# MarSaKi/VLN-BEVBert

Hardware: AMD Instinct MI355X
Metric: pretrain_samples_per_sec (higher is better)
Workload: dtype bf16+fp32-residual

## Files before the change

### include/bevbert_hip.h

```cpp
#ifndef BEVBERT_HIP_H
#define BEVBERT_HIP_H

#include <stdint.h>

#ifdef __cplusplus
extern "C" {
#endif

typedef struct ihipStream_t* hipStream_t;

#define BEVBERT_F32 0
#define BEVBERT_BF16 1
#define BEVBERT_F16 2

const char* bevbert_last_error(void);
int bevbert_version(void);
int bevbert_hip_error_reset(void);
const char* bevbert_arch(void);
const char* bevbert_attn_last_path(int backward);
const char* bevbert_attn_plan(int B, int nh, int Lq, int Lk, int dtype, int impl, int has_key_mask, int has_bias,
                              float drop_p, int has_bits, int bits_ready, int want_dbias, int ncu, int backward);

int bevbert_bev_lift_bin(const float* depths, const float* T_c2w, const float* T_w2c, const float* S_w2c,
                         const float* pix_scale, int B, int V, int hw, float depth_scale, int dim, float res,
// ... 38 lines not shown
                                const float* gamma, const float* beta, void* y16, float* y32, float* z32, float* mean,
                                float* rstd, int rows, int H, float eps, float drop_p, uint64_t seed, uint64_t offset,
                                hipStream_t stream);
int bevbert_layernorm_res32_bwd(const void* dy16, const float* dy32, const float* z32, const float* mean,
                                const float* rstd, const float* gamma, void* dz, void* dx16, float* dgamma,
                                float* dbeta, float* dbias, float* workspace, int rows, int H, float drop_p, uint64_t seed,
                                uint64_t offset, int accumulate, int dz_dtype,
                                hipStream_t stream);
int64_t bevbert_colsum_workspace_floats(int total_cols);
int bevbert_colsum_partial_rows(int rows);
int bevbert_colsum_finalize(const float* partials, int nblocks, int nwhich, int C, float* out0, float* out1,
                            float* out2, int accumulate, hipStream_t stream);
int bevbert_colsum_partials(const void* dy, float* partials, int rows, int C, int dtype, hipStream_t stream);
int bevbert_multi_finalize(const void* tasks, int ntasks, hipStream_t stream);
int bevbert_multi_accum(const void* tasks, int ntasks, hipStream_t stream);

int bevbert_embed_sum_layernorm_fwd(const int64_t* ids, const void* word, const void* pos, const void* type_row,
                                    const float* gamma, const float* beta, void* y, void* z_out, float* mean,
                                    float* rstd, int rows, int L, int H, float eps, int dtype, float drop_p,
                                    uint64_t seed, uint64_t offset, hipStream_t stream);

int bevbert_embedding_grad(const int64_t* ids, const void* d, float* table_grad, int rows, int H, int padding_idx,
                           int dtype, hipStream_t stream);

int64_t bevbert_smallk_workspace_floats(int rows, int K, int H);
int bevbert_smallk_linear_layernorm_fwd(const float* feat, const float* weight, const float* bias, const float* gamma,
                                        const float* beta, const void* post1, const void* table, const int64_t* idx,
                                        void* y, float* mean, float* rstd, int rows, int K, int H, float eps, int dtype,
                                        hipStream_t stream);
int bevbert_smallk_linear_layernorm_bwd(const void* dy, const float* feat, const float* weight, const float* bias,
// ... 28 lines not shown

int bevbert_bias_gelu_fwd(const void* x, const float* bias, void* y, int rows, int C, int dtype, hipStream_t stream);
int bevbert_bias_gelu_bwd(const void* dy, const void* x, const float* bias, void* dx, float* dbias, float* workspace,
                          int rows, int C, int dtype, int accumulate, hipStream_t stream);
int bevbert_bias_relu_fwd(const void* x, const float* bias, void* y, int rows, int C, int dtype, hipStream_t stream);
int bevbert_bias_relu_bwd(const void* dy, const void* x, const float* bias, void* dx, float* dbias, float* workspace,
                          int rows, int C, int dtype, int accumulate, hipStream_t stream);
int bevbert_colsum(const void* dy, float* out, float* workspace, int rows, int C, int dtype, int accumulate,
                   hipStream_t stream);

int bevbert_segment_wsum(const void* src, const int* rowptr, const int* idx, const float* w, void* out, int out_rows,
                         int H, int dtype, hipStream_t stream);

int bevbert_grad_norm_clip(const float* grads, int64_t n, float pre_scale, float max_norm, float* partials,
                           float* scalars, hipStream_t stream);
int bevbert_adamw_step(float* params, const float* grads, float* exp_avg, float* exp_avg_sq, void* params_bf16,
                       const uint8_t* chunk_flags, int* chunk_steps, int64_t n, const float* grad_scale_dev,
                       const float* lr_dev, float lr, float beta1, float beta2, float eps, float weight_decay,
                       hipStream_t stream);
int bevbert_cast_f32(const float* src, void* dst, int64_t n, int dst_dtype, hipStream_t stream);
int bevbert_zero(void* p, int64_t bytes, hipStream_t stream);
int bevbert_accum_partials(const void* partials, float* sink, int S, int64_t n, int dtype, hipStream_t stream);

int bevbert_gemm(const void* A, const void* B, void* C, const void* bias, int M, int N, int K, int opA, int opB,
                 int64_t lda, int64_t ldb, int64_t ldc, int batch, int64_t stride_a, int64_t stride_b,
                 int64_t stride_c, int in_dtype, int out_dtype, int bias_dtype, float alpha, void* workspace,
                 int64_t workspace_bytes, int autotune, hipStream_t stream);
int bevbert_gemm_plan(int M, int N, int K, int opA, int opB, int64_t lda, int64_t ldb, int64_t ldc, int batch,
                      int64_t stride_a, int64_t stride_b, int64_t stride_c, int in_dtype, int out_dtype, int bias_dtype,
                      int accumulate, int64_t workspace_bytes, int autotune);
// ... 216 lines not shown
```

### vln_bevbert_amd/arena.py

```python
import math

import torch

from . import lib
from .lib import ptr, stream


def call(name, *args):
    from . import ops
    return ops.call(name, *args)

CHUNK = 1024
_ZERO_KERNEL = __import__("os").environ.get("BEVBERT_ZERO_KERNEL", "0") == "1"
NO_DECAY = ("bias", "LayerNorm.bias", "LayerNorm.weight")


def _round_up(n, m):
    return (n + m - 1) // m * m


class ParamArena:
    def __init__(self, module, device, compute_dtype=torch.float32, groups=()):
        self.device = torch.device(device)
        self.compute_dtype = compute_dtype
        named = [(n, p) for n, p in module.named_parameters()]
        by_name = dict(named)
        in_group = {}
        for gi, g in enumerate(groups):
            for n in g:
                in_group[n] = gi
        layout, seen_groups = [], set()
        for n, p in named:
            if n in in_group:
                gi = in_group[n]
                if gi in seen_groups:
                    continue
# ... 43 lines not shown
        self._param_versions = None
        self.step_count = 0
        self._scalars = torch.zeros(4, dtype=torch.float32, device=dev)
        self._partials = torch.zeros(1024, dtype=torch.float32, device=dev)
        self.named = named
        for n, p in named:
            o, k = self.slices[n]
            view = self.params[o:o + k].view(p.shape)
            view.copy_(p.data.to(dev, torch.float32))
            p.data = view
            p.main_grad = self.grads[o:o + k].view(p.shape)
            p.compute = self.shadow[o:o + k].view(p.shape) if self.shadow is not None else p.data
            p.arena = self
            p.arena_name = n
        self._index = {n: i for i, (n, _) in enumerate(named)}
        self.sync_shadow()
        self._param_versions = sum(p._version for _, p in named)

    def packed(self, names, shape):
        o0, _ = self.slices[names[0]]
        total = 0
        for n in names:
            o, k = self.slices[n]
            assert o == o0 + total, f"{names} are not contiguous in the arena"
            total += k
        assert total == math.prod(shape)
        src = self.shadow if self.shadow is not None else self.params
        return src[o0:o0 + total].view(shape), self.grads[o0:o0 + total].view(shape)

    def touch(self, param):
# ... 61 lines not shown
        if self.shadow is not None:
            call("bevbert_cast_f32", ptr(self.params), ptr(self.shadow), self.numel, lib.dtype_code(self.compute_dtype),
                 stream())

    def sync(self):
        if self.device.type == "cuda":
            from . import ops
            ops.WgradStream.flush_all()
            cur = torch.cuda.current_stream(self.device)
            for side in ops.Branches.side_streams():
                if ops.Branches.enabled or side not in ops.WgradStream.streams or ops.WgradStream.dirty:
                    cur.wait_stream(side)
            ops.WgradStream.dirty = False
            ops.WgradStream.release()

    def backward_done(self):
        self.sync()

    def zero_grad(self, overlap=False):
        self.sync()
        if self.device.type == "cuda":
            from . import ops
            ops.RT.scratch.reset()
            if overlap:
                if getattr(self, "_zero_stream", None) is None:
                    from .hwqueues import side_stream
                    self._zero_stream = side_stream(self.device)
                self._zero_stream.wait_stream(torch.cuda.current_stream(self.device))
                with torch.cuda.stream(self._zero_stream):
                    if _ZERO_KERNEL:
                        self.grads.zero_()
                    else:
                        call("bevbert_zero", ptr(self.grads), self.grads.numel() * 4, stream())
                self._zero_pending = True
                return
            call("bevbert_zero", ptr(self.grads), self.grads.numel() * 4, stream())
            return
        self.grads.zero_()
# ... 5 lines not shown

    def load_state_dict_into(self, module, sd, strict=True):
        out = module.load_state_dict(sd, strict=strict)
        self.sync_shadow()
        return out

    def set_lr(self, lr):
        self._scalars[2:3].fill_(float(lr))
        self._lr_set = True

    def upload_flags(self):
        if self._flags_dirty:
            self.flags.copy_(self._flags_host, non_blocking=True)
            self._flags_dirty = False

    def clip_and_step(self, lr=None, betas=(0.9, 0.98), eps=1e-6, weight_decay=0.01, max_norm=5.0, grad_pre_scale=1.0):
        self.sync()
        if self.exp_avg is None:
            self.exp_avg = torch.zeros_like(self.params)
            self.exp_avg_sq = torch.zeros_like(self.params)
        if lr is not None:
            self.set_lr(lr)
        elif not getattr(self, "_lr_set", False):
            raise RuntimeError("clip_and_step(lr=None) reads the device-resident learning rate: call set_lr() first "
                               "(the slot starts at 0, which would silently turn AdamW and its weight decay into a no-op)")
        if not torch.cuda.is_current_stream_capturing():
            self.upload_flags()
        self.step_count += 1
        call("bevbert_grad_norm_clip", ptr(self.grads), self.numel, float(grad_pre_scale),
             float(max_norm if max_norm is not None else -1.0), ptr(self._partials), ptr(self._scalars), stream())
        call("bevbert_adamw_step", ptr(self.params), ptr(self.grads), ptr(self.exp_avg), ptr(self.exp_avg_sq),
             ptr(self.shadow), ptr(self.flags), ptr(self.chunk_steps), self.numel, self._scalars[1:].data_ptr(),
             self._scalars[2:].data_ptr(), 0.0, float(betas[0]), float(betas[1]), float(eps), float(weight_decay),
             stream())

    def grad_norm(self):
        return self._scalars[0]
```

### vln_bevbert_amd/csrc/capi.hip

```cpp
#include <stdarg.h>

#include "attn_common.h"

static thread_local char g_err[512] = "";

void bb_set_error(const char* fmt, ...) {
  va_list ap;
  va_start(ap, fmt);
  vsnprintf(g_err, sizeof(g_err), fmt, ap);
  va_end(ap);
}

BEVBERT_API const char* bevbert_last_error(void) { return g_err; }
BEVBERT_API int bevbert_hip_error_reset(void) {
  int n = 0;
  while (hipGetLastError() != hipSuccess && n < 16) ++n;
  return n;
}

BEVBERT_API int bevbert_zero(void* p, int64_t bytes, hipStream_t stream) {
  BB_REQUIRE(p != nullptr && bytes >= 0, "zero: null pointer or negative size");
  if (bytes == 0) return BB_OK;
  hipError_t e = hipMemsetAsync(p, 0, (size_t)bytes, stream);
  if (e != hipSuccess) {
    bb_set_error("zero: hipMemsetAsync failed: %s", hipGetErrorString(e));
    return BB_ELAUNCH;
  }
  return BB_OK;
}

BEVBERT_API int bevbert_version(void) { return 205; }

static const uint32_t* g_step_salt = nullptr;
const uint32_t* bb_step_salt() { return g_step_salt; }
BEVBERT_API int bevbert_set_step_salt(const void* device_word) {
  g_step_salt = static_cast<const uint32_t*>(device_word);
  return BB_OK;
}
BEVBERT_API const char* bevbert_arch(void) { return "gfx950"; }

int attn_simple_fwd(const AttnArgs& a, int dtype, hipStream_t st);
int attn_simple_bwd(const AttnArgs& a, int dtype, hipStream_t st);
int attn_delta(const AttnArgs& a, float* delta, int dtype, hipStream_t st);
int attn_mfma_fwd(const AttnArgs& a, hipStream_t st);
int attn_mfma_bwd(const AttnArgs& a, hipStream_t st);
int attn_mfma_bwd1(const AttnArgs& a, hipStream_t st);
bool attn_mfma_bwd1_supported(const AttnArgs& a);
int attn_fwd2(const AttnArgs& a, hipStream_t st);
bool attn_fwd2_supported(const AttnArgs& a);
int attn_drop_bits(const AttnArgs& a, uint64_t* bits_f, uint64_t* bits_b, uint32_t* bits_l, hipStream_t st);
int attn_fwd4(const AttnArgs& a, const uint32_t* bits_l, hipStream_t st);
// ... 259 lines not shown
```

### vln_bevbert_amd/csrc/common.h

```cpp
#pragma once
#include <hip/hip_runtime.h>
#include <hip/hip_bf16.h>
#include <stdint.h>
#include <stdio.h>
#include <string.h>
#include <type_traits>

#include "../../include/bevbert_hip.h"

#define BEVBERT_API extern "C" __attribute__((visibility("default")))

enum { BB_F32 = BEVBERT_F32, BB_BF16 = BEVBERT_BF16, BB_F16 = BEVBERT_F16 };

enum { BB_OK = 0, BB_EINVAL = -1, BB_ELAUNCH = -2, BB_EUNSUPPORTED = -3 };

void bb_set_error(const char* fmt, ...);

#define BB_REQUIRE(cond, ...)            \
  do {                                   \
    if (!(cond)) {                       \
      bb_set_error(__VA_ARGS__);         \
      return BB_EINVAL;                  \
    }                                    \
  } while (0)
// ... 134 lines not shown
__host__ __device__ __forceinline__ uint32_t bb_site_key(uint64_t seed, uint64_t offset) {
  uint32_t k = bb_hash32((uint32_t)seed ^ 0x9e3779b9u);
  k = bb_hash32(k ^ (uint32_t)(seed >> 32));
  k = bb_hash32(k ^ (uint32_t)offset);
  return bb_hash32(k ^ (uint32_t)(offset >> 32));
}
constexpr uint32_t BB_STREAM_NAV = 0x6e617631u, BB_STREAM_WAYPOINT = 0x77617970u, BB_STREAM_GHOST = 0x67687374u;
constexpr uint32_t BB_STREAM_CE_ACTION = 0x63656163u;
__host__ __device__ __forceinline__ uint32_t bb_stream_key(uint32_t key, uint32_t domain) { return bb_hash32(key ^ domain); }
__host__ __device__ __forceinline__ uint32_t bb_drop_threshold(float p) {
  const float t = p * 65536.0f + 0.5f;
  if (t <= 0.f) return 0u;
  return t >= 65535.f ? 65535u : (uint32_t)t;
}
const uint32_t* bb_step_salt();
__device__ __forceinline__ uint32_t bb_salted(uint32_t key, const uint32_t* __restrict__ salt) {
  return salt ? bb_hash32(key ^ *salt) : key;
}
__device__ __forceinline__ uint32_t bb_pair_bits(uint32_t key, uint32_t pair_idx) { return bb_hash32(pair_idx ^ key); }
__device__ __forceinline__ bool bb_keep_lo(uint32_t bits, uint32_t thr) { return (bits & 0xffffu) >= thr; }
__device__ __forceinline__ bool bb_keep_hi(uint32_t bits, uint32_t thr) { return (bits >> 16) >= thr; }
__device__ __forceinline__ bool bb_keep(uint32_t key, uint32_t idx, uint32_t thr) {
  const uint32_t bits = bb_pair_bits(key, idx >> 1);
  return ((idx & 1u) ? (bits >> 16) : (bits & 0xffffu)) >= thr;
}
__device__ __forceinline__ float4 bb_drop4(float4 v, uint32_t elem, uint32_t key, uint32_t thr, float keep_scale) {
  const uint32_t pr = elem >> 1;
  const uint32_t b0 = bb_pair_bits(key, pr), b1 = bb_pair_bits(key, pr + 1);
  v.x = bb_keep_lo(b0, thr) ? v.x * keep_scale : 0.f;
  v.y = bb_keep_hi(b0, thr) ? v.y * keep_scale : 0.f;
// ... 66 lines not shown
```

### vln_bevbert_amd/csrc/rowops.hip

```cpp
#include <math.h>
#include <type_traits>

#include "common.h"

__device__ __forceinline__ float4 ln_fwd_input(float4 a, const float* __restrict__ bias, int col, float drop_p, uint32_t elem,
                                               uint32_t drop_key, uint32_t drop_thr, float keep_scale, bool has_res,
                                               const float4 r) {
  if (bias != nullptr) add4(a, *reinterpret_cast<const float4*>(bias + col));
  if (drop_p > 0.f) a = bb_drop4(a, elem, drop_key, drop_thr, keep_scale);
  if (has_res) add4(a, r);
  return a;
}

template <typename T, int NV, bool GATHER>
__global__ __launch_bounds__(256) void ln_fwd_kernel(const T* __restrict__ x, const float* __restrict__ bias,
                                                     const T* __restrict__ residual, const float* __restrict__ gamma,
                                                     const float* __restrict__ beta, T* __restrict__ y,
                                                     T* __restrict__ z_out, float* __restrict__ mean_out,
                                                     float* __restrict__ rstd_out, int rows, float eps, float drop_p,
                                                     uint32_t drop_thr, uint32_t drop_key,
                                                     const int64_t* __restrict__ ids, const T* __restrict__ word,
                                                     const T* __restrict__ pos, const T* __restrict__ type_row, int L,
                                                     const uint32_t* __restrict__ salt) {
  constexpr int H = NV * 256;
// ... 529 lines not shown
  const int r = blockIdx.x;
  const int e0 = rowptr[r], e1 = rowptr[r + 1];
  for (int c = threadIdx.x * 4; c < H; c += blockDim.x * 4) {
    float4 acc = make_float4(0.f, 0.f, 0.f, 0.f);
    for (int e = e0; e < e1; ++e) {
      const float ww = w[e];
      const float4 v = ld4<T>(src + (size_t)idx[e] * H + c);
      acc.x += ww * v.x; acc.y += ww * v.y; acc.z += ww * v.z; acc.w += ww * v.w;
    }
    st4<T>(out + (size_t)r * H + c, acc);
  }
}

#define ACCUM_U 4
#define ACCUM_SC 4
template <typename T>
__device__ __forceinline__ void accum_fold(const T* part_, float* sink_, size_t stride4, size_t n4, int S, size_t first,
                                           size_t step) {
  const BB_GLOBAL T* __restrict__ part = (const BB_GLOBAL T*)part_;
  BB_GLOBAL float* __restrict__ sink = (BB_GLOBAL float*)sink_;
  for (size_t i = first; i < n4; i += ACCUM_U * step) {
    size_t idx[ACCUM_U];
    float4 acc[ACCUM_U];
#pragma unroll
    for (int u = 0; u < ACCUM_U; ++u) {
      idx[u] = i + u * step < n4 ? i + u * step : n4 - 1;
      acc[u] = gld4<float>(sink + idx[u] * 4);
    }
    int s = 0;
    for (; s + ACCUM_SC <= S; s += ACCUM_SC) {
      float4 v[ACCUM_SC][ACCUM_U];
#pragma unroll
      for (int k = 0; k < ACCUM_SC; ++k)
#pragma unroll
        for (int u = 0; u < ACCUM_U; ++u) v[k][u] = gld4<T>(part + ((size_t)(s + k) * stride4 + idx[u]) * 4);
#pragma unroll
      for (int k = 0; k < ACCUM_SC; ++k)
#pragma unroll
        for (int u = 0; u < ACCUM_U; ++u) add4(acc[u], v[k][u]);
    }
    for (; s < S; ++s) {
      float4 v[ACCUM_U];
#pragma unroll
      for (int u = 0; u < ACCUM_U; ++u) v[u] = gld4<T>(part + ((size_t)s * stride4 + idx[u]) * 4);
#pragma unroll
      for (int u = 0; u < ACCUM_U; ++u) add4(acc[u], v[u]);
    }
#pragma unroll
    for (int u = 0; u < ACCUM_U; ++u)
      if (i + u * step < n4) {
        const bb_f4v o = {acc[u].x, acc[u].y, acc[u].z, acc[u].w};
        *reinterpret_cast<BB_GLOBAL bb_f4v*>(sink + idx[u] * 4) = o;
      }
  }
}

template <typename T>
__global__ __launch_bounds__(256) void accum_partials_kernel(const T* __restrict__ partials, float* __restrict__ sink,
                                                             int S, size_t n4) {
  accum_fold<T>(partials, sink, n4, n4, S, (size_t)blockIdx.x * 256 + threadIdx.x, (size_t)gridDim.x * 256);
}

struct AccumTask {
  const void* partials;
  float* sink;
  unsigned long long n4_total;
  unsigned int off4, n4;
  int S, dtype;
};
template <typename T>
__device__ __forceinline__ void accum_task(const AccumTask& t) {
  accum_fold<T>((const T*)t.partials + (size_t)t.off4 * 4, t.sink, t.n4_total, t.n4, t.S, threadIdx.x, 256);
}
__global__ __launch_bounds__(256) void multi_accum_kernel(const AccumTask* __restrict__ tasks) {
  const AccumTask t = tasks[blockIdx.x];
  if (t.dtype == BB_BF16) accum_task<bf16_raw>(t);
  else accum_task<float>(t);
}

#define EG_MAXJ 4
template <typename T, typename TO = float, bool ACCUM = true>
__global__ __launch_bounds__(256) void embedding_grad_kernel(const int64_t* __restrict__ ids, const T* __restrict__ d,
                                                             TO* __restrict__ table_grad, int rows, int H,
                                                             int padding_idx) {
  __shared__ int s_flag;
  __shared__ float s_part[4][256 * EG_MAXJ];
  const int r = blockIdx.x, tid = threadIdx.x, lane = tid & 63, wave = tid >> 6;
  const int64_t id = ids[r];
  if (id == (int64_t)padding_idx) return;
  if (tid == 0) s_flag = 0;
  __syncthreads();
  int hit = 0;
// ... 71 lines not shown
    *reinterpret_cast<float4*>(partials + ((size_t)s * ntab + t) * H + c) = acc;
  }
}

__global__ __launch_bounds__(256) void sumsq_kernel(const float* __restrict__ g, size_t n4, float* __restrict__ partials) {
  float s = 0.f;
  for (size_t i = (size_t)blockIdx.x * 256 + threadIdx.x; i < n4; i += (size_t)gridDim.x * 256) {
    const float4 v = *reinterpret_cast<const float4*>(g + i * 4);
    s += (v.x * v.x + v.y * v.y) + (v.z * v.z + v.w * v.w);
  }
  __shared__ float sh[4];
  s = wave_sum(s);
  if ((threadIdx.x & 63) == 0) sh[threadIdx.x >> 6] = s;
  __syncthreads();
  if (threadIdx.x == 0) partials[blockIdx.x] = (sh[0] + sh[1]) + (sh[2] + sh[3]);
}

__global__ void clip_coef_kernel(const float* __restrict__ partials, int n, float pre_scale, float max_norm,
                                 float* __restrict__ scalars) {
  __shared__ double sh[256];
  double s = 0.0;
  for (int i = threadIdx.x; i < n; i += 256) s += (double)partials[i];
  sh[threadIdx.x] = s;
  __syncthreads();
  for (int o = 128; o > 0; o >>= 1) {
    if (threadIdx.x < o) sh[threadIdx.x] += sh[threadIdx.x + o];
    __syncthreads();
  }
  if (threadIdx.x == 0) {
    const float norm = (float)sqrt(sh[0]) * pre_scale;
// ... 579 lines not shown
  const int nb = colwise_blocks(rows);
  const dim3 grid(nb, (C + 1023) / 1024);
  const bool type_ok = bb_with_type(dtype, [&](auto t) {
    using T = decltype(t);
    hipLaunchKernelGGL((colwise_bwd_kernel<T, 1>), grid, dim3(256), 0, stream, (const T*)dy, nullptr, nullptr, nullptr, partials, rows, C);
  });
  if (!type_ok) return bb_dtype_unsupported("colsum_partials", dtype);
  BB_CHECK_LAUNCH("colsum_partials");
  return BB_OK;
}

BEVBERT_API int bevbert_multi_accum(const void* tasks, int ntasks, hipStream_t stream) {
  static_assert(sizeof(AccumTask) == 40, "AccumTask is part of the C ABI");
  if (ntasks <= 0) return BB_OK;
  BB_REQUIRE(tasks != nullptr, "multi_accum: null task table");
  hipLaunchKernelGGL(multi_accum_kernel, dim3(ntasks), dim3(256), 0, stream, (const AccumTask*)tasks);
  BB_CHECK_LAUNCH("multi_accum");
  return BB_OK;
}

BEVBERT_API int bevbert_multi_finalize(const void* tasks, int ntasks, hipStream_t stream) {
  static_assert(sizeof(FinalizeTask) == 40, "FinalizeTask is part of the C ABI");
  if (ntasks <= 0) return BB_OK;
  BB_REQUIRE(tasks != nullptr, "multi_finalize: null task table");
  hipLaunchKernelGGL(multi_finalize_kernel, dim3(ntasks), dim3(64, 16), 0, stream, (const FinalizeTask*)tasks);
  BB_CHECK_LAUNCH("multi_finalize");
  return BB_OK;
}

BEVBERT_API int bevbert_segment_wsum(const void* src, const int* rowptr, const int* idx, const float* w, void* out,
                                     int out_rows, int H, int dtype, hipStream_t stream) {
  BB_REQUIRE(H % 4 == 0, "segment_wsum: H=%d must be a multiple of 4", H);
// ... 77 lines not shown
    using T = decltype(t);
    hipLaunchKernelGGL(embedding_grad_sliced_kernel<T>, grid, dim3(nt), 0, stream, ids, (const T*)d, partials, rows, H, rows_per_slice,
                       table_rows);
  });
  if (!type_ok) return bb_dtype_unsupported("embedding_grad_sliced", dtype);
  BB_CHECK_LAUNCH("embedding_grad_sliced");
  return BB_OK;
}

BEVBERT_API int bevbert_grad_norm_clip(const float* grads, int64_t n, float pre_scale, float max_norm,
                                       float* partials, float* scalars, hipStream_t stream) {
  BB_REQUIRE(n % 4 == 0, "grad_norm_clip: n must be a multiple of 4");
  hipLaunchKernelGGL(sumsq_kernel, dim3(1024), dim3(256), 0, stream, grads, (size_t)n / 4, partials);
  hipLaunchKernelGGL(clip_coef_kernel, dim3(1), dim3(256), 0, stream, partials, 1024, pre_scale, max_norm, scalars);
  BB_CHECK_LAUNCH("grad_norm_clip");
  return BB_OK;
}

BEVBERT_API int bevbert_adamw_step(float* params, const float* grads, float* exp_avg, float* exp_avg_sq,
                                   void* params_bf16, const uint8_t* chunk_flags, int* chunk_steps, int64_t n,
                                   const float* grad_scale_dev, const float* lr_dev, float lr, float beta1,
                                   float beta2, float eps, float weight_decay, hipStream_t stream) {
  BB_REQUIRE(n % 1024 == 0, "adamw_step: arena length must be a multiple of 1024 elements");
  BB_REQUIRE(chunk_steps != nullptr, "adamw_step: per-chunk step counters are required");
  const size_t nchunks = (size_t)n / 1024;
  hipLaunchKernelGGL(adamw_kernel, dim3(nchunks), dim3(256), 0, stream, params, grads, exp_avg, exp_avg_sq,
                     (bf16_raw*)params_bf16, chunk_flags, chunk_steps, nchunks, grad_scale_dev, lr_dev, lr, beta1, beta2, eps,
                     weight_decay, (float)log2((double)beta1), (float)log2((double)beta2));
  BB_CHECK_LAUNCH("adamw_step");
  return BB_OK;
// ... 45 lines not shown
```

### vln_bevbert_amd/ops_reduce.py

```python
import math
import os as _os

import torch

from . import lib
from .lib import stream
from .ops_core import ATTN_BITS, Branches, RT, call


def join_captured_side_streams(extra=()):
    if not torch.cuda.is_available() or not torch.cuda.is_current_stream_capturing():
        return 0
    cur = torch.cuda.current_stream()
    seen, n = {cur.cuda_stream}, 0
    cands = [ATTN_BITS.stream] + list(Branches._streams.values()) + list(WgradStream.streams) + list(extra)
    for st in cands:
        if st is None or st.cuda_stream in seen:
            continue
        seen.add(st.cuda_stream)
        with torch.cuda.stream(st):
            capturing = torch.cuda.is_current_stream_capturing()
        if capturing:
            cur.wait_stream(st)
            n += 1
# ... 182 lines not shown

ScratchRing.INITIAL = int(_os.environ.get("BEVBERT_SCRATCH_INITIAL_MB", "256")) << 20
RT.scratch = SCRATCH


class ReduceQueue:

    jobs = []
    accum_jobs = []
    table_bytes = {}
    producers = {}
    _tables = {}
    _accum_tables = {}
    _dtype = None
    _adtype = None

    @classmethod
    def _note_producer(cls):
        st = WgradStream._target
        if st is None:
            if not torch.cuda.is_available():
                return
            st = torch.cuda.current_stream()
        cls.producers[st.cuda_stream] = st

    @classmethod
    def wait_producers(cls, consumer):
        for h, st in cls.producers.items():
            if h != consumer.cuda_stream:
                consumer.wait_stream(st)
        cls.producers = {}

    @classmethod
    def drop_pending(cls):
        cls.jobs, cls.accum_jobs, cls.producers = [], [], {}

    @classmethod
    def add_accum(cls, partials_ptr, sink_ptr, S, n, dtype):
        cls.accum_jobs.append((partials_ptr, sink_ptr, S, n, dtype))
        cls._note_producer()

    @classmethod
    def _build_accum(cls, jobs, device):
        import numpy as np
        if cls._adtype is None:
            cls._adtype = np.dtype([("partials", "<u8"), ("sink", "<u8"), ("n4_total", "<u8"), ("off4", "<u4"),
                                    ("n4", "<u4"), ("S", "<i4"), ("dtype", "<i4")])
        parts = []
        for partials_ptr, sink_ptr, S, n, dt in jobs:
            n4 = n // 4
            off = np.arange(0, n4, 4096, dtype=np.int64)
            t = np.zeros(len(off), dtype=cls._adtype)
            t["partials"] = partials_ptr
            t["sink"] = sink_ptr + off * 16
            t["n4_total"] = n4
            t["off4"] = off
            t["n4"] = np.minimum(4096, n4 - off)
            t["S"] = S
            t["dtype"] = dt
            parts.append(t)
        table = np.concatenate(parts) if parts else np.zeros(0, dtype=cls._adtype)
        dev = torch.from_numpy(table.view(np.uint8).copy()).to(device)
        cls.table_bytes[dev.data_ptr()] = int(sum(S * n * (4 if dt == lib.F32 else 2) + 8 * n for _, _, S, n, dt in jobs))
        return dev, len(table)

    @classmethod
    def add(cls, partials_ptr, nblocks, nwhich, C, outs, accumulate=1):
        cls.jobs.append((partials_ptr, nblocks, nwhich, C, outs[0] or 0, outs[1] or 0, outs[2] or 0, accumulate))
        cls._note_producer()

    @classmethod
    def _build(cls, jobs, device):
        import numpy as np
        if cls._dtype is None:
            cls._dtype = np.dtype([("partials", "<u8"), ("out", "<u8"), ("nblocks", "<i4"), ("row_stride", "<i4"),
                                   ("col0", "<i4"), ("ncols", "<i4"), ("accumulate", "<i4"), ("pad", "<i4")])
        parts = []
        for partials_ptr, nblocks, nwhich, C, o0, o1, o2, acc in jobs:
            ntile = (C + 63) // 64
# ... 7 lines not shown
                t["nblocks"] = nblocks
                t["row_stride"] = nwhich * C
                t["col0"] = which * C + tiles * 64
                t["ncols"] = np.minimum(64, C - tiles * 64)
                t["accumulate"] = acc
                parts.append(t)
        table = np.concatenate(parts) if parts else np.zeros(0, dtype=cls._dtype)
        dev = torch.from_numpy(table.view(np.uint8).copy()).to(device)
        cls.table_bytes[dev.data_ptr()] = int(4 * (table["nblocks"].astype(np.int64) * table["ncols"]).sum()
                                              + 4 * (table["ncols"] * (1 + (table["accumulate"] != 0))).sum()) if len(table) else 0
        return dev, len(table)

    @classmethod
    def flush(cls, device):
        if cls.accum_jobs:
            akey = tuple(cls.accum_jobs)
            cls.accum_jobs = []
            aent = cls._accum_tables.get(akey)
            if aent is None:
                if torch.cuda.is_current_stream_capturing():
                    raise lib.BevBertHipError("accumulate task table missing during graph capture (warm-up steps build it)")
                if len(cls._accum_tables) > 256:
                    cls._accum_tables.clear()
                rounds, seen = [[]], [set()]
                for job in akey:
                    r = 0
                    while job[1] in seen[r]:
                        r += 1
                        if r == len(rounds):
                            rounds.append([])
                            seen.append(set())
                    rounds[r].append(job)
                    seen[r].add(job[1])
                aent = cls._accum_tables[akey] = [cls._build_accum(tuple(r), device) for r in rounds]
            for table, n in aent:
                call("bevbert_multi_accum", table.data_ptr(), n, stream())
        if not cls.jobs:
            return
        key = tuple(cls.jobs)
        cls.jobs = []
        ent = cls._tables.get(key)
        if ent is None:
            if torch.cuda.is_current_stream_capturing():
                raise lib.BevBertHipError("reduction task table missing during graph capture (warm-up steps build it)")
            if len(cls._tables) > 256:
                cls._tables.clear()
            rounds, seen = [[]], [set()]
            for job in key:
                outs = {o for o in job[4:7] if o}
                r = 0
                while outs & seen[r]:
# ... 27 lines not shown
```

### vln_bevbert_amd/train.py

```python
import os
import random

import torch
import torch.distributed as dist

from . import ops
from .static_step import GraphedStep, StaticBatch


def warmup_linear_lr(step, base_lr, warmup_steps, total_steps):
    f = step / warmup_steps if step < warmup_steps else max(0, (total_steps - step) / (total_steps - warmup_steps))
    lr = base_lr * f
    return lr if lr > 0 else 1e-8


def load_gemm_tuning():
    import os
    path = os.path.join(os.path.dirname(os.path.abspath(__file__)), "tunableop_results.csv")
    if os.environ.get("BEVBERT_GEMM_TUNING", "1") != "1" or not os.path.exists(path):
        return 0
    try:
        import torch.cuda.tunable as tunable
        tunable.enable(True)
        tunable.tuning_enable(False)
# ... 182 lines not shown
        if self.active and not self._phase_a_done:
            self._phase_a_done = True
            self.launch_uncovered(self.split, self.flat.numel())

    def finish(self):
        if self.active:
            for lo, hi in self._remaining():
                self._launch(lo, hi)
            for w in self._works:
                w.wait()
            if self.stream is not None:
                torch.cuda.current_stream().wait_stream(self.stream)
        self._works = []
        self._phase_a_done = False
        self._done = []


class PretrainTrainer:
    def __init__(self, model, arena, learning_rate=5e-5, warmup_steps=10000, num_train_steps=100000,
                 betas=(0.9, 0.98), weight_decay=0.01, grad_norm=5.0, seed=0, rank=0, world_size=1, overlap=True,
                 force_collectives=False):
        self.model, self.arena = model, arena
        arena.publish_grads = False
        self.lr, self.warmup, self.total = learning_rate, warmup_steps, num_train_steps
        self.betas, self.wd, self.grad_norm = betas, weight_decay, grad_norm
        self.seed, self.rank, self.world = seed, rank, world_size
        self.global_step = 0
        import os
        self.use_graphs = os.environ.get("BEVBERT_GRAPHS", "1") == "1" and arena.device.type == "cuda"
        self.graph_branches = os.environ.get("BEVBERT_GRAPH_BRANCHES", "1") == "1"
# ... 3 lines not shown
        first_map = min(arena.slices[n][0] for n in arena.slices
                        if n.startswith("bert.local_encoder") or n.startswith("bert.global_encoder")
                        or not n.startswith("bert."))
        self.reducer = GradReducer(arena.grads, first_map, force=force_collectives)
        self.reducer.set_occupied(arena.slices.values())
        self.reducer.settle_collective_queue()
        self.overlap = overlap and self.reducer.active
        self.capture_ok = not (self.reducer.active and self.reducer.exchange == "bf16_a2a")
        if self.reducer.active and dist.get_backend(self.reducer.group) != "nccl":
            self.capture_ok = False
        if self.reducer.active:
            self.broadcast_state()
        self.early_flush = os.environ.get("BEVBERT_EARLY_FLUSH", "0") == "1" and arena.device.type == "cuda"
        if self.early_flush and not self.overlap:
            model.bert.lang_encoder.register_forward_hook(self._hook_flush)
        if self.overlap:
            self.install_map_layer_hooks()
            model.bert.lang_encoder.register_forward_hook(self._hook_text)
            for k, lo, hi in self.text_layer_regions(model, arena):
                model.bert.lang_encoder.layer[k].register_forward_pre_hook(self._make_layer_hook(lo, hi))

    @staticmethod
    def map_layer_regions(model, arena):
        out = {}
        heads = [(o, o + k) for n, (o, k) in arena.slices.items() if not n.startswith("bert.")]
        if heads:
            lo, hi = min(lo for lo, _ in heads), max(hi for _, hi in heads)
            if not any(n.startswith("bert.") and lo <= o < hi for n, (o, c) in arena.slices.items()):
                out["heads"] = (lo, hi)
        for enc in ("local", "global"):
# ... 107 lines not shown
            self.arena.wait_zero()
        if self.reducer is not None and self.reducer.timeline is not None:
            self.backward_start = torch.cuda.Event(enable_timing=True)
            self.backward_start.record()
        if loss.is_cuda and loss.dim() == 0:
            one = self.__dict__.get("_one")
            if one is None or one.dtype != loss.dtype or one.device != loss.device:
                one = self._one = torch.ones((), dtype=loss.dtype, device=loss.device)
            loss.backward(gradient=one)
        else:
            loss.backward()
        self.arena.sync()
        self.reducer.finish()
        return loss.detach()

    def optimizer_step(self, lr=None):
        if lr is None:
            lr = warmup_linear_lr(self.global_step, self.lr, self.warmup, self.total)
        self.arena.clip_and_step(lr, self.betas, 1e-6, self.wd, self.grad_norm, grad_pre_scale=1.0 / self.world)

    def step(self, task, batch):
        if isinstance(batch, StaticBatch) and self.use_graphs and self.capture_ok and batch.capturable and ops.RT.trace is None:
            return self._static_step(task, batch)
        loss = self.forward_backward(task, batch)
        self.optimizer_step()
        return loss

    def validate(self, val_loaders, setname="", **kw):
        from .validate import validate
        return validate(self.model, val_loaders, setname, **kw)

    GRAPH_WARMUP = 2

    def _static_step(self, task, sb):
        assert sb.task == task
        self.global_step += 1
        lr = warmup_linear_lr(self.global_step, self.lr, self.warmup, self.total)
        a = self.arena
        if a.exp_avg is None:
            a.exp_avg = torch.zeros_like(a.params)
# ... 2 lines not shown
                        else self._plan_key(task, sb))
        a.set_lr(lr)
        gs = sb.graph
        if gs is not None and gs.owner is self:
            a.upload_flags()
            gs.graph.replay()
            return gs.loss.clone()
        branches = ops.Branches.enabled
        if sb.eager_runs < self.GRAPH_WARMUP:
            sb.eager_runs += 1
            ops.Branches.enabled = branches or self.graph_branches
            try:
                loss = self._forward_backward(task, sb)
            finally:
                ops.Branches.enabled = branches
            self.optimizer_step(lr=None)
            return loss
        a.upload_flags()
        torch.cuda.synchronize()
        graph = torch.cuda.CUDAGraph()
        if self._graph_pool is None:
            self._graph_pool = torch.cuda.graph_pool_handle()
        ops.Branches.enabled = branches or self.graph_branches
        mode = "thread_local"
        if self.reducer.active:
            import time
            time.sleep(0.3)
        err = None
        try:
            with torch.cuda.graph(graph, pool=self._graph_pool, capture_error_mode=mode):
                try:
                    ops.RT.new_step(0, write_salt=False, plan_key=self._plan_key(task, sb))
                    loss = self._forward_backward(task, sb)
                    a.clip_and_step(None, self.betas, 1e-6, self.wd, self.grad_norm, grad_pre_scale=1.0 / self.world)
                except Exception as e:
                    err = e
                    ops.join_captured_side_streams(extra=[self.reducer.stream])
        except Exception as e:
            err = err or e
        if err is not None:
            e = err
            import warnings
            self.graph_error = f"{type(e).__name__}: {e}"[:400]
            self.use_graphs = False
            warnings.warn(f"hipGraph capture of the {task} step failed, continuing with eager steps: {self.graph_error}")
            ops.Branches.enabled = branches
            from . import lib
            lib.load().bevbert_hip_error_reset()
            if torch.cuda.is_current_stream_capturing():
                raise RuntimeError("the failed hipGraph capture could not be ended: the stream is still capturing and the "
                                   f"process cannot issue work any more ({self.graph_error})") from e
            torch.cuda.synchronize()
            ops.WgradStream.drop_pending()
            ops.ReduceQueue.drop_pending()
            self.reducer.drop_pending()
            ops.RT.new_step(self._step_seed(), plan_key=self._plan_key(task, sb))
            loss = self._forward_backward(task, sb)
            self.optimizer_step(lr=None)
            return loss
        ops.Branches.enabled = branches
        gs = GraphedStep(graph, loss)
        gs.owner = self
        sb.graph = gs
        graph.replay()
        return loss.clone()


class ArenaDataParallel(torch.nn.Module):

    def __init__(self, module, process_group=None, compute_dtype=None):
        super().__init__()
        self.module = module
        arena = getattr(module, "arena", None)
# ... 36 lines not shown
```

Baseline: 3641.

## Fuse gradient-norm partial sums into split-K fold and store-mode accumulation

The split-K fold kernel now optionally overwrites its sink instead of reading and adding, which saves a load of the zeroed arena gradient. It also emits per-block sums of squares into a registered slot array. A small complement kernel sums the squares of the arena ranges not covered by the folds. The clip coefficient is then computed from those slots, replacing the full-arena norm pass. This removes one full read of the gradient buffer before AdamW. The cost is extra bookkeeping, validation checks on the first run, and a reliance on no other writer touching the folded gradients after the fold.

```diff
diff --git a/include/bevbert_hip.h b/include/bevbert_hip.h
--- a/include/bevbert_hip.h
+++ b/include/bevbert_hip.h
@@ -76,6 +76,8 @@
 int bevbert_colsum_partials(const void* dy, float* partials, int rows, int C, int dtype, hipStream_t stream);
 int bevbert_multi_finalize(const void* tasks, int ntasks, hipStream_t stream);
 int bevbert_multi_accum(const void* tasks, int ntasks, hipStream_t stream);
+int bevbert_set_fold_norm_slots(float* slots, int capacity);
+int bevbert_sumsq_tasks(const void* tasks, int ntasks, hipStream_t stream);
 
 int bevbert_embed_sum_layernorm_fwd(const int64_t* ids, const void* word, const void* pos, const void* type_row,
                                     const float* gamma, const float* beta, void* y, void* z_out, float* mean,
@@ -134,6 +136,8 @@
 
 int bevbert_grad_norm_clip(const float* grads, int64_t n, float pre_scale, float max_norm, float* partials,
                            float* scalars, hipStream_t stream);
+int bevbert_clip_from_slots(const float* slots, int n, float pre_scale, float max_norm, float* scalars,
+                            hipStream_t stream);
 int bevbert_adamw_step(float* params, const float* grads, float* exp_avg, float* exp_avg_sq, void* params_bf16,
                        const uint8_t* chunk_flags, int* chunk_steps, int64_t n, const float* grad_scale_dev,
                        const float* lr_dev, float lr, float beta1, float beta2, float eps, float weight_decay,
diff --git a/vln_bevbert_amd/arena.py b/vln_bevbert_amd/arena.py
--- a/vln_bevbert_amd/arena.py
+++ b/vln_bevbert_amd/arena.py
@@ -20,6 +20,8 @@
 
 
 class ParamArena:
+    _serial = 0
+
     def __init__(self, module, device, compute_dtype=torch.float32, groups=()):
         self.device = torch.device(device)
         self.compute_dtype = compute_dtype
@@ -93,6 +95,18 @@
             p.arena = self
             p.arena_name = n
         self._index = {n: i for i, (n, _) in enumerate(named)}
+        self.fold_store = False
+        ParamArena._serial += 1
+        self.fold_key = ("arena", ParamArena._serial)
+        tables = {id(m.weight) for m in module.modules() if isinstance(m, torch.nn.Embedding)}
+        self._fold_ranges = []
+        for o, k, _ in sorted((*self.slices[n], n) for n, p in named if p.dim() >= 2 and id(p) not in tables):
+            if self._fold_ranges and self._fold_ranges[-1][1] == o:
+                self._fold_ranges[-1][1] = o + k
+            else:
+                self._fold_ranges.append([o, o + k])
+        self._fold_starts = [a for a, _ in self._fold_ranges]
+        self._fold_comp = {}
         self.sync_shadow()
         self._param_versions = sum(p._version for _, p in named)
 
@@ -184,6 +198,97 @@
             ops.WgradStream.dirty = False
             ops.WgradStream.release()
 
+    def store_ok(self, sink_ptr, n):
+        import bisect
+        off, rem = divmod(sink_ptr - self.grads.data_ptr(), 4)
+        if rem or off < 0 or off + n > self.numel:
+            return False
+        i = bisect.bisect_right(self._fold_starts, off) - 1
+        return i >= 0 and off + n <= self._fold_ranges[i][1]
+
+    def _arm_fold(self):
+        from . import ops
+        ops.ReduceQueue.store_ok = self.store_ok if self.fold_store else None
+        ops.ReduceQueue.fold_norm = None
+
+    def _name_at(self, sink_ptr):
+        off = (sink_ptr - self.grads.data_ptr()) // 4
+        return next((n for n, (o, k) in self.slices.items() if o <= off < o + k), f"arena offset {off}")
+
+    def fold_check_zero(self, stores):
+        base = self.grads.data_ptr()
+        views = [self.grads[(p - base) // 4:(p - base) // 4 + n] for p, n in stores]
+        counts = torch.stack([torch.count_nonzero(v) for v in views]).tolist()
+        bad = [(self._name_at(p), c) for (p, _), c in zip(stores, counts) if c]
+        if bad:
+            raise lib.BevBertHipError(
+                "store-mode fold: the gradient of " + ", ".join(f"{n} ({c} non-zero elements)" for n, c in bad[:4])
+                + " is not zero before the step's fold -- something other than the split-K fold writes it, or the arena "
+                "was not zeroed for this step (BEVBERT_FOLD_STORE=0 turns the store mode off)")
+
+    def _fold_complement(self, entry):
+        ent = self._fold_comp.get(id(entry))
+        if ent is not None and ent[0] is entry:
+            return ent[1:]
+        if torch.cuda.is_current_stream_capturing():
+            raise lib.BevBertHipError("fold-norm complement table missing during graph capture (warm-up steps build it)")
+        import numpy as np
+        base, recs, pos = self.grads.data_ptr(), [], 0
+        for p, n, _ in sorted(entry["norm_jobs"]) + [(base + 4 * self.numel, 0, 0)]:
+            o = (p - base) // 4
+            for a in range(pos, o, 16384):
+                recs.append((base + 4 * a, (min(a + 16384, o) - a) // 4))
+            pos = o + n
+            assert pos % 4 == 0, "fold sinks are float4-aligned"
+        from . import ops
+        if entry["nslots"] + len(recs) > ops.ReduceQueue.SLOT_CAPACITY:
+            return None
+        t = np.zeros(len(recs), dtype=np.dtype([("ptr", "<u8"), ("n4", "<u4"), ("slot", "<u4")]))
+        if recs:
+            t["ptr"], t["n4"] = zip(*recs)
+        t["slot"] = entry["nslots"] + np.arange(len(recs))
+        dev = torch.from_numpy(t.view(np.uint8).copy()).to(self.device)
+        if len(self._fold_comp) > 64:
+            self._fold_comp.clear()
+        self._fold_comp[id(entry)] = (entry, dev, len(recs), 16 * int(t["n4"].sum()))
+        return dev, len(recs), 16 * int(t["n4"].sum())
+
+    def _clip_from_fold(self, pre_scale, max_norm):
+        from . import ops
+        rec, ops.ReduceQueue.fold_norm = ops.ReduceQueue.fold_norm, None
+        if rec is None or rec["owner"] is not self:
+            return False
+        entry = rec["entry"]
+        comp = self._fold_complement(entry)
+        if comp is None:
+            return False
+        table, ntasks, _ = comp
+        slots = ops.ReduceQueue.register_slots(self.device)
+        call("bevbert_sumsq_tasks", table.data_ptr(), ntasks, stream())
+        call("bevbert_clip_from_slots", ptr(slots), entry["nslots"] + ntasks, pre_scale, max_norm, ptr(self._scalars),
+             stream())
+        if entry["fresh"] and not torch.cuda.is_current_stream_capturing():
+            entry["fresh"] = False
+            self._fold_check_norm(entry, slots, pre_scale)
+        return True
+
+    def _fold_check_norm(self, entry, slots, pre_scale):
+        want = float(torch.linalg.vector_norm(self.grads, dtype=torch.float64)) * pre_scale
+        got = float(self._scalars[0])
+        if abs(got - want) <= 1e-5 * want or (got == 0.0 and want == 0.0):
+            return
+        base, culprit = self.grads.data_ptr(), "a range outside the folds"
+        for p, n, s0 in entry["norm_jobs"]:
+            o = (p - base) // 4
+            w = float(self.grads[o:o + n].double().pow(2).sum())
+            g = float(slots[s0:s0 + (n // 4 + 4095) // 4096].double().sum())
+            if abs(g - w) > 1e-5 * max(w, 1e-30):
+                culprit = self._name_at(p)
+                break
+        raise lib.BevBertHipError(
+            f"fused gradient norm {got!r} differs from the arena's {want!r}: the gradient of {culprit} changed after the "
+            "step's fold (BEVBERT_FOLD_STORE=0 turns the fused norm off)")
+
     def backward_done(self):
         self.sync()
 
@@ -192,6 +297,7 @@
         if self.device.type == "cuda":
             from . import ops
             ops.RT.scratch.reset()
+            self._arm_fold()
             if overlap:
                 if getattr(self, "_zero_stream", None) is None:
                     from .hwqueues import side_stream
@@ -227,7 +333,8 @@
             self.flags.copy_(self._flags_host, non_blocking=True)
             self._flags_dirty = False
 
-    def clip_and_step(self, lr=None, betas=(0.9, 0.98), eps=1e-6, weight_decay=0.01, max_norm=5.0, grad_pre_scale=1.0):
+    def clip_and_step(self, lr=None, betas=(0.9, 0.98), eps=1e-6, weight_decay=0.01, max_norm=5.0, grad_pre_scale=1.0,
+                      fused_norm=False):
         self.sync()
         if self.exp_avg is None:
             self.exp_avg = torch.zeros_like(self.params)
@@ -240,8 +347,10 @@
         if not torch.cuda.is_current_stream_capturing():
             self.upload_flags()
         self.step_count += 1
-        call("bevbert_grad_norm_clip", ptr(self.grads), self.numel, float(grad_pre_scale),
-             float(max_norm if max_norm is not None else -1.0), ptr(self._partials), ptr(self._scalars), stream())
+        max_norm = float(max_norm if max_norm is not None else -1.0)
+        if not (fused_norm and self._clip_from_fold(float(grad_pre_scale), max_norm)):
+            call("bevbert_grad_norm_clip", ptr(self.grads), self.numel, float(grad_pre_scale), max_norm,
+                 ptr(self._partials), ptr(self._scalars), stream())
         call("bevbert_adamw_step", ptr(self.params), ptr(self.grads), ptr(self.exp_avg), ptr(self.exp_avg_sq),
              ptr(self.shadow), ptr(self.flags), ptr(self.chunk_steps), self.numel, self._scalars[1:].data_ptr(),
              self._scalars[2:].data_ptr(), 0.0, float(betas[0]), float(betas[1]), float(eps), float(weight_decay),
diff --git a/vln_bevbert_amd/csrc/capi.hip b/vln_bevbert_amd/csrc/capi.hip
--- a/vln_bevbert_amd/csrc/capi.hip
+++ b/vln_bevbert_amd/csrc/capi.hip
@@ -35,6 +35,18 @@
 const uint32_t* bb_step_salt() { return g_step_salt; }
 BEVBERT_API int bevbert_set_step_salt(const void* device_word) {
   g_step_salt = static_cast<const uint32_t*>(device_word);
+  return BB_OK;
+}
+static float* g_fold_norm_slots = nullptr;
+static int g_fold_norm_capacity = 0;
+float* bb_fold_norm_slots(int* capacity) {
+  *capacity = g_fold_norm_capacity;
+  return g_fold_norm_slots;
+}
+BEVBERT_API int bevbert_set_fold_norm_slots(float* slots, int capacity) {
+  BB_REQUIRE(capacity >= 0 && capacity <= (1 << 20), "set_fold_norm_slots: capacity %d outside [0, 2^20]", capacity);
+  g_fold_norm_slots = capacity > 0 ? slots : nullptr;
+  g_fold_norm_capacity = g_fold_norm_slots ? capacity : 0;
   return BB_OK;
 }
 BEVBERT_API const char* bevbert_arch(void) { return "gfx950"; }
diff --git a/vln_bevbert_amd/csrc/common.h b/vln_bevbert_amd/csrc/common.h
--- a/vln_bevbert_amd/csrc/common.h
+++ b/vln_bevbert_amd/csrc/common.h
@@ -172,6 +172,7 @@
   return t >= 65535.f ? 65535u : (uint32_t)t;
 }
 const uint32_t* bb_step_salt();
+float* bb_fold_norm_slots(int* capacity);
 __device__ __forceinline__ uint32_t bb_salted(uint32_t key, const uint32_t* __restrict__ salt) {
   return salt ? bb_hash32(key ^ *salt) : key;
 }
diff --git a/vln_bevbert_amd/csrc/rowops.hip b/vln_bevbert_amd/csrc/rowops.hip
--- a/vln_bevbert_amd/csrc/rowops.hip
+++ b/vln_bevbert_amd/csrc/rowops.hip
@@ -567,18 +567,20 @@
 
 #define ACCUM_U 4
 #define ACCUM_SC 4
-template <typename T>
-__device__ __forceinline__ void accum_fold(const T* part_, float* sink_, size_t stride4, size_t n4, int S, size_t first,
-                                           size_t step) {
+template <typename T, bool STORE = false>
+__device__ __forceinline__ float accum_fold(const T* part_, float* sink_, size_t stride4, size_t n4, int S, size_t first,
+                                            size_t step) {
   const BB_GLOBAL T* __restrict__ part = (const BB_GLOBAL T*)part_;
   BB_GLOBAL float* __restrict__ sink = (BB_GLOBAL float*)sink_;
+  float sq = 0.f;
   for (size_t i = first; i < n4; i += ACCUM_U * step) {
     size_t idx[ACCUM_U];
     float4 acc[ACCUM_U];
 #pragma unroll
     for (int u = 0; u < ACCUM_U; ++u) {
       idx[u] = i + u * step < n4 ? i + u * step : n4 - 1;
-      acc[u] = gld4<float>(sink + idx[u] * 4);
+      if constexpr (STORE) acc[u] = make_float4(0.f, 0.f, 0.f, 0.f);
+      else acc[u] = gld4<float>(sink + idx[u] * 4);
     }
     int s = 0;
     for (; s + ACCUM_SC <= S; s += ACCUM_SC) {
@@ -604,8 +606,10 @@
       if (i + u * step < n4) {
         const bb_f4v o = {acc[u].x, acc[u].y, acc[u].z, acc[u].w};
         *reinterpret_cast<BB_GLOBAL bb_f4v*>(sink + idx[u] * 4) = o;
+        sq += (acc[u].x * acc[u].x + acc[u].y * acc[u].y) + (acc[u].z * acc[u].z + acc[u].w * acc[u].w);
       }
   }
+  return sq;
 }
 
 template <typename T>
@@ -621,14 +625,31 @@
   unsigned int off4, n4;
   int S, dtype;
 };
-template <typename T>
-__device__ __forceinline__ void accum_task(const AccumTask& t) {
-  accum_fold<T>((const T*)t.partials + (size_t)t.off4 * 4, t.sink, t.n4_total, t.n4, t.S, threadIdx.x, 256);
-}
-__global__ __launch_bounds__(256) void multi_accum_kernel(const AccumTask* __restrict__ tasks) {
+#define ACCUM_STORE 0x100
+#define ACCUM_NORM 0x200
+__device__ __forceinline__ float block_sum_256(float s) {
+  __shared__ float sh[4];
+  s = wave_sum(s);
+  if ((threadIdx.x & 63) == 0) sh[threadIdx.x >> 6] = s;
+  __syncthreads();
+  return (sh[0] + sh[1]) + (sh[2] + sh[3]);
+}
+template <typename T, bool STORE>
+__device__ __forceinline__ float accum_task(const AccumTask& t) {
+  return accum_fold<T, STORE>((const T*)t.partials + (size_t)t.off4 * 4, t.sink, t.n4_total, t.n4, t.S, threadIdx.x, 256);
+}
+__global__ __launch_bounds__(256) void multi_accum_kernel(const AccumTask* __restrict__ tasks, float* __restrict__ slots,
+                                                          unsigned int capacity) {
   const AccumTask t = tasks[blockIdx.x];
-  if (t.dtype == BB_BF16) accum_task<bf16_raw>(t);
-  else accum_task<float>(t);
+  const bool bf16 = (t.dtype & 0xff) == BB_BF16;
+  float sq;
+  if (t.dtype & ACCUM_STORE) sq = bf16 ? accum_task<bf16_raw, true>(t) : accum_task<float, true>(t);
+  else sq = bf16 ? accum_task<bf16_raw, false>(t) : accum_task<float, false>(t);
+  const unsigned int slot = (unsigned int)t.dtype >> 12;
+  if ((t.dtype & ACCUM_NORM) && slot < capacity) {
+    sq = block_sum_256(sq);
+    if (threadIdx.x == 0) slots[slot] = sq;
+  }
 }
 
 #define EG_MAXJ 4
@@ -730,6 +751,32 @@
   if ((threadIdx.x & 63) == 0) sh[threadIdx.x >> 6] = s;
   __syncthreads();
   if (threadIdx.x == 0) partials[blockIdx.x] = (sh[0] + sh[1]) + (sh[2] + sh[3]);
+}
+
+struct SumsqTask {
+  const float* ptr;
+  unsigned int n4, slot;
+};
+__global__ __launch_bounds__(256) void sumsq_tasks_kernel(const SumsqTask* __restrict__ tasks, float* __restrict__ slots,
+                                                          unsigned int capacity) {
+  const SumsqTask t = tasks[blockIdx.x];
+  if (t.slot >= capacity) return;
+  const unsigned int n4 = t.n4 < 4096u ? t.n4 : 4096u;
+  float s = 0.f;
+  if (n4) {
+    const BB_GLOBAL float* __restrict__ g = (const BB_GLOBAL float*)t.ptr;
+    float4 v[16];
+#pragma unroll
+    for (int u = 0; u < 16; ++u) {
+      const unsigned int i = threadIdx.x + u * 256;
+      v[u] = gld4<float>(g + (size_t)(i < n4 ? i : n4 - 1) * 4);
+    }
+#pragma unroll
+    for (int u = 0; u < 16; ++u)
+      if (threadIdx.x + u * 256 < n4) s += (v[u].x * v[u].x + v[u].y * v[u].y) + (v[u].z * v[u].z + v[u].w * v[u].w);
+  }
+  s = block_sum_256(s);
+  if (threadIdx.x == 0) slots[t.slot] = s;
 }
 
 __global__ void clip_coef_kernel(const float* __restrict__ partials, int n, float pre_scale, float max_norm,
@@ -1339,8 +1386,23 @@
   static_assert(sizeof(AccumTask) == 40, "AccumTask is part of the C ABI");
   if (ntasks <= 0) return BB_OK;
   BB_REQUIRE(tasks != nullptr, "multi_accum: null task table");
-  hipLaunchKernelGGL(multi_accum_kernel, dim3(ntasks), dim3(256), 0, stream, (const AccumTask*)tasks);
+  int capacity = 0;
+  float* slots = bb_fold_norm_slots(&capacity);
+  hipLaunchKernelGGL(multi_accum_kernel, dim3(ntasks), dim3(256), 0, stream, (const AccumTask*)tasks, slots,
+                     (unsigned int)(slots ? capacity : 0));
   BB_CHECK_LAUNCH("multi_accum");
+  return BB_OK;
+}
+
+BEVBERT_API int bevbert_sumsq_tasks(const void* tasks, int ntasks, hipStream_t stream) {
+  static_assert(sizeof(SumsqTask) == 16, "SumsqTask is part of the C ABI");
+  if (ntasks <= 0) return BB_OK;
+  int capacity = 0;
+  float* slots = bb_fold_norm_slots(&capacity);
+  BB_REQUIRE(tasks != nullptr && slots != nullptr, "sumsq_tasks: null task table, or no slot array registered");
+  hipLaunchKernelGGL(sumsq_tasks_kernel, dim3(ntasks), dim3(256), 0, stream, (const SumsqTask*)tasks, slots,
+                     (unsigned int)capacity);
+  BB_CHECK_LAUNCH("sumsq_tasks");
   return BB_OK;
 }
 
@@ -1448,6 +1510,14 @@
   hipLaunchKernelGGL(sumsq_kernel, dim3(1024), dim3(256), 0, stream, grads, (size_t)n / 4, partials);
   hipLaunchKernelGGL(clip_coef_kernel, dim3(1), dim3(256), 0, stream, partials, 1024, pre_scale, max_norm, scalars);
   BB_CHECK_LAUNCH("grad_norm_clip");
+  return BB_OK;
+}
+
+BEVBERT_API int bevbert_clip_from_slots(const float* slots, int n, float pre_scale, float max_norm, float* scalars,
+                                        hipStream_t stream) {
+  BB_REQUIRE(n >= 0 && (slots != nullptr || n == 0) && scalars != nullptr, "clip_from_slots: null pointer or negative count");
+  hipLaunchKernelGGL(clip_coef_kernel, dim3(1), dim3(256), 0, stream, slots, n, pre_scale, max_norm, scalars);
+  BB_CHECK_LAUNCH("clip_from_slots");
   return BB_OK;
 }
 
diff --git a/vln_bevbert_amd/ops_reduce.py b/vln_bevbert_amd/ops_reduce.py
--- a/vln_bevbert_amd/ops_reduce.py
+++ b/vln_bevbert_amd/ops_reduce.py
@@ -220,6 +220,26 @@
     _accum_tables = {}
     _dtype = None
     _adtype = None
+    FOLD_STORE = _os.environ.get("BEVBERT_FOLD_STORE", "1") == "1"
+    STORE, NORM = 0x100, 0x200
+    SLOT_CAPACITY = 1 << 16
+    store_ok = None
+    fold_norm = None
+    _slots = None
+
+    @classmethod
+    def slots(cls, device):
+        if cls._slots is None:
+            if torch.cuda.is_current_stream_capturing():
+                raise lib.BevBertHipError("fold-norm slot array missing during graph capture (warm-up steps allocate it)")
+            cls._slots = torch.zeros(cls.SLOT_CAPACITY, dtype=torch.float32, device=device)
+        return cls._slots
+
+    @classmethod
+    def register_slots(cls, device):
+        s = cls.slots(device)
+        lib.load().bevbert_set_fold_norm_slots(s.data_ptr(), s.numel())
+        return s
 
     @classmethod
     def _note_producer(cls):
@@ -247,13 +267,14 @@
         cls._note_producer()
 
     @classmethod
-    def _build_accum(cls, jobs, device):
+    def _build_accum(cls, jobs, device, flags=None, slot0=0):
         import numpy as np
         if cls._adtype is None:
             cls._adtype = np.dtype([("partials", "<u8"), ("sink", "<u8"), ("n4_total", "<u8"), ("off4", "<u4"),
                                     ("n4", "<u4"), ("S", "<i4"), ("dtype", "<i4")])
-        parts = []
-        for partials_ptr, sink_ptr, S, n, dt in jobs:
+        parts, slot = [], slot0
+        flags = flags if flags is not None else [0] * len(jobs)
+        for (partials_ptr, sink_ptr, S, n, dt), fl in zip(jobs, flags):
             n4 = n // 4
             off = np.arange(0, n4, 4096, dtype=np.int64)
             t = np.zeros(len(off), dtype=cls._adtype)
@@ -263,12 +284,45 @@
             t["off4"] = off
             t["n4"] = np.minimum(4096, n4 - off)
             t["S"] = S
-            t["dtype"] = dt
+            word = np.full(len(off), dt | (fl & (cls.STORE | cls.NORM)), dtype=np.int64)
+            if fl & cls.NORM:
+                word |= (slot + np.arange(len(off), dtype=np.int64)) << 12
+                slot += len(off)
+            t["dtype"] = word.astype(np.uint32).view(np.int32)
             parts.append(t)
         table = np.concatenate(parts) if parts else np.zeros(0, dtype=cls._adtype)
         dev = torch.from_numpy(table.view(np.uint8).copy()).to(device)
-        cls.table_bytes[dev.data_ptr()] = int(sum(S * n * (4 if dt == lib.F32 else 2) + 8 * n for _, _, S, n, dt in jobs))
+        cls.table_bytes[dev.data_ptr()] = int(sum(S * n * (4 if dt == lib.F32 else 2) + (4 * n if fl & cls.STORE else 8 * n)
+                                                  for (_, _, S, n, dt), fl in zip(jobs, flags)))
         return dev, len(table)
+
+    @classmethod
+    def _plan_fold(cls, jobs, ok):
+        rounds, seen, last = [[]], [set()], {}
+        for job in jobs:
+            r = 0
+            while job[1] in seen[r]:
+                r += 1
+                if r == len(rounds):
+                    rounds.append([])
+                    seen.append(set())
+            rounds[r].append(job)
+            seen[r].add(job[1])
+            last[job[1]] = r
+        if ok is None:
+            return rounds, [[0] * len(r) for r in rounds]
+        lengths = {}
+        for job in jobs:
+            lengths.setdefault(job[1], set()).add(job[3])
+        spans = sorted((p, p + 4 * max(ns)) for p, ns in lengths.items())
+        clash = set()
+        for (p0, e0), (p1, _) in zip(spans, spans[1:]):
+            if e0 > p1:
+                clash |= {p0, p1}
+        good = {p for p, ns in lengths.items() if len(ns) == 1 and p not in clash and ok(p, next(iter(ns)))}
+        flags = [[(cls.STORE if r == 0 and j[1] in good else 0) | (cls.NORM if j[1] in good and last[j[1]] == r else 0)
+                  for j in rnd] for r, rnd in enumerate(rounds)]
+        return rounds, flags
 
     @classmethod
     def add(cls, partials_ptr, nblocks, nwhich, C, outs, accumulate=1):
@@ -306,27 +360,42 @@
     @classmethod
     def flush(cls, device):
         if cls.accum_jobs:
-            akey = tuple(cls.accum_jobs)
+            jobs = tuple(cls.accum_jobs)
             cls.accum_jobs = []
+            ok, cls.store_ok, cls.fold_norm = (cls.store_ok if cls.FOLD_STORE else None), None, None
+            owner = getattr(ok, "__self__", ok)
+            akey = (jobs, None if ok is None else getattr(owner, "fold_key", id(owner)))
             aent = cls._accum_tables.get(akey)
             if aent is None:
                 if torch.cuda.is_current_stream_capturing():
                     raise lib.BevBertHipError("accumulate task table missing during graph capture (warm-up steps build it)")
                 if len(cls._accum_tables) > 256:
                     cls._accum_tables.clear()
-                rounds, seen = [[]], [set()]
-                for job in akey:
-                    r = 0
-                    while job[1] in seen[r]:
-                        r += 1
-                        if r == len(rounds):
-                            rounds.append([])
-                            seen.append(set())
-                    rounds[r].append(job)
-                    seen[r].add(job[1])
-                aent = cls._accum_tables[akey] = [cls._build_accum(tuple(r), device) for r in rounds]
-            for table, n in aent:
+                rounds, flags = cls._plan_fold(jobs, ok)
+                tasks_of = lambda j: (j[3] // 4 + 4095) // 4096
+                n_norm = sum(tasks_of(j) for rnd, fl in zip(rounds, flags) for j, f in zip(rnd, fl) if f & cls.NORM)
+                if n_norm > cls.SLOT_CAPACITY // 2:
+                    flags = [[f & ~cls.NORM for f in fl] for fl in flags]
+                tables, nslots, norm_jobs = [], 0, []
+                for rnd, fl in zip(rounds, flags):
+                    tables.append(cls._build_accum(tuple(rnd), device, fl, nslots))
+                    for j, f in zip(rnd, fl):
+                        if f & cls.NORM:
+                            norm_jobs.append((j[1], j[3], nslots))
+                            nslots += tasks_of(j)
+                aent = {
+                    "tables": tables, "nslots": nslots, "norm_jobs": norm_jobs, "fresh": True,
+                    "flagged": any(f for fl in flags for f in fl),
+                    "stores": [(j[1], j[3]) for rnd, fl in zip(rounds, flags) for j, f in zip(rnd, fl) if f & cls.STORE]}
+                if aent["stores"] and hasattr(owner, "fold_check_zero"):
+                    _on_launch_stream(lambda: owner.fold_check_zero(aent["stores"]))
+                cls._accum_tables[akey] = aent
+            if aent["flagged"]:
+                cls.register_slots(device)
+            for table, n in aent["tables"]:
                 call("bevbert_multi_accum", table.data_ptr(), n, stream())
+            if aent["nslots"]:
+                cls.fold_norm = {"owner": owner, "entry": aent}
         if not cls.jobs:
             return
         key = tuple(cls.jobs)
diff --git a/vln_bevbert_amd/train.py b/vln_bevbert_amd/train.py
--- a/vln_bevbert_amd/train.py
+++ b/vln_bevbert_amd/train.py
@@ -220,6 +220,11 @@
         self._works = []
         self._phase_a_done = False
         self._done = []
+
+
+def fold_store_allowed(device_type, reducer_active, early_flush, env=None):
+    env = os.environ if env is None else env
+    return env.get("BEVBERT_FOLD_STORE", "1") == "1" and device_type == "cuda" and not reducer_active and not early_flush
 
 
 class PretrainTrainer:
@@ -253,6 +258,7 @@
         self.early_flush = os.environ.get("BEVBERT_EARLY_FLUSH", "0") == "1" and arena.device.type == "cuda"
         if self.early_flush and not self.overlap:
             model.bert.lang_encoder.register_forward_hook(self._hook_flush)
+        arena.fold_store = fold_store_allowed(arena.device.type, self.reducer.active, self.early_flush)
         if self.overlap:
             self.install_map_layer_hooks()
             model.bert.lang_encoder.register_forward_hook(self._hook_text)
@@ -390,16 +396,17 @@
         self.reducer.finish()
         return loss.detach()
 
-    def optimizer_step(self, lr=None):
+    def optimizer_step(self, lr=None, fused_norm=False):
         if lr is None:
             lr = warmup_linear_lr(self.global_step, self.lr, self.warmup, self.total)
-        self.arena.clip_and_step(lr, self.betas, 1e-6, self.wd, self.grad_norm, grad_pre_scale=1.0 / self.world)
+        self.arena.clip_and_step(lr, self.betas, 1e-6, self.wd, self.grad_norm, grad_pre_scale=1.0 / self.world,
+                                 fused_norm=fused_norm)
 
     def step(self, task, batch):
         if isinstance(batch, StaticBatch) and self.use_graphs and self.capture_ok and batch.capturable and ops.RT.trace is None:
             return self._static_step(task, batch)
         loss = self.forward_backward(task, batch)
-        self.optimizer_step()
+        self.optimizer_step(fused_norm=True)
         return loss
 
     def validate(self, val_loaders, setname="", **kw):
@@ -432,7 +439,7 @@
                 loss = self._forward_backward(task, sb)
             finally:
                 ops.Branches.enabled = branches
-            self.optimizer_step(lr=None)
+            self.optimizer_step(lr=None, fused_norm=True)
             return loss
         a.upload_flags()
         torch.cuda.synchronize()
@@ -450,7 +457,8 @@
                 try:
                     ops.RT.new_step(0, write_salt=False, plan_key=self._plan_key(task, sb))
                     loss = self._forward_backward(task, sb)
-                    a.clip_and_step(None, self.betas, 1e-6, self.wd, self.grad_norm, grad_pre_scale=1.0 / self.world)
+                    a.clip_and_step(None, self.betas, 1e-6, self.wd, self.grad_norm, grad_pre_scale=1.0 / self.world,
+                                    fused_norm=True)
                 except Exception as e:
                     err = e
                     ops.join_captured_side_streams(extra=[self.reducer.stream])
@@ -474,7 +482,7 @@
             self.reducer.drop_pending()
             ops.RT.new_step(self._step_seed(), plan_key=self._plan_key(task, sb))
             loss = self._forward_backward(task, sb)
-            self.optimizer_step(lr=None)
+            self.optimizer_step(lr=None, fused_norm=True)
             return loss
         ops.Branches.enabled = branches
         gs = GraphedStep(graph, loss)
```

Result: faster. 3697 (median of 6 runs) (+1.5%).
